# hsp-iit/roft

Hardware: AMD Instinct MI355X
Metric: tracker frames/sec per object (640x480) + ADD-S vs CPU ref (higher is better)
Workload: dtype f64; 1 GPU; BASELINE config #4: 640x480, CV_32FC2 flow grid 1, 64 objects in total, 64 per GPU (sharded by object, no data-path collective; result rows all-gathered over RCCL at N > 1), masks+poses at 5 fps with 6-frame delay, flow-aided masks, re-sync and outlier rejection on, frames submitted in batches of at most 8; objects_per_gpu=64, objects_total=64, width=640, height=480, batch_frames=8, ranks=1, backend=nccl

## Files before the change

### roft_amd/csrc/engine.hip

```cpp
#include "engine_internal.h"

namespace {
thread_local std::string g_last_error;
}

namespace roft {
namespace host {
int fail(int code, const std::string& msg)
{
    g_last_error = msg;
    return code;
}
}
}
const std::string& last_error() { return g_last_error; }

namespace roft {
int device_cu_count()
{
    static std::mutex mu;
    static std::vector<int> cus;
    int dev = 0;
    if (hipGetDevice(&dev) != hipSuccess || dev < 0) return 256;
    std::lock_guard<std::mutex> lk(mu);
// ... 635 lines not shown
            if (e->objs[obj_ids[i]]->s.track_frames > 0)
                HIP_TRY(hipMemcpyAsync(&last[i], e->arr.state.p + obj_ids[i], sizeof(ObjState), hipMemcpyDeviceToHost, s));
        HIP_TRY(hipStreamSynchronize(s));
    }
    long long meshes = 0;
    for (int i = 0; i < n; ++i) {
        const int id = obj_ids[i];
        HostObject* o = e->objs[id].get();
        if (running && o->s.track_frames > 0) {
            const ObjState& st = last[i];
            roft_object_output& out = o->last_out;
            std::memcpy(out.pose, st.belief[B_LIN0 + o->stepped_slot].mean, sizeof(double) * 13);
            std::memcpy(out.twist, st.v_mean, sizeof(double) * 6);
            out.n_flow_points = st.n_flow_points;
            out.outlier_selected = st.lane[o->stepped_lane].outlier_selected;
            out.outlier_L[0] = st.lane[o->stepped_lane].outlier_L[0];
            out.outlier_L[1] = st.lane[o->stepped_lane].outlier_L[1];
            o->last_out_valid = true;
        }
        bool mesh_uploaded = false;
        TRY(apply_object_desc(e, id, o, &descs[i], keep_mesh, &fresh[i], s, &mesh_uploaded));
        meshes += mesh_uploaded ? 1 : 0;
        o->owned.clear();
        o->s = Sched();
        o->s.frame_idx = e->frame_counter;
        o->stepped_slot = o->stepped_lane = 0;
        o->stepped_flow = nullptr;
        o->stepped_depth = nullptr;
        if (!running) continue;
        HIP_TRY(hipMemsetAsync(e->arr.planes.p + plane_offset(a, id, 0, 0), 0, sizeof(uint32_t) * (size_t)kPlaneSlotsTotal * 2 * a.plane_words, s));
        HIP_TRY(hipMemset2DAsync(e->arr.mrec.p + id, sizeof(MaskRec) * (size_t)a.n_obj, 0, sizeof(MaskRec), (size_t)2 * (kMaxBatch + 1), s));
        HIP_TRY(hipMemsetAsync(e->arr.mask_general.p + id, 0, sizeof(unsigned), s));
        HIP_TRY(hipMemset2DAsync(e->arr.npts.p + id, sizeof(int) * (size_t)a.n_obj, 0, sizeof(int), (size_t)e->T_max, s));
    }
    HIP_TRY(hipStreamSynchronize(s));
    update_mesh_maxima(e, n_obj);
    e->restart_stats.calls++;
    e->restart_stats.objects += n;
    e->restart_stats.meshes_replaced += meshes;
    return ROFT_OK;
}

int roft_engine_get_restart_stats(roft_engine* e, roft_engine_restart_stats* out)
{
    if (!e || !out) return fail(ROFT_ERR_INVALID, "null argument");
    *out = e->restart_stats;
    return ROFT_OK;
}
```

### roft_amd/csrc/engine_internal.h

```cpp
#pragma once

#include <hip/hip_runtime.h>

#include <algorithm>
#include <cfloat>
#include <chrono>
#include <cmath>
#include <cstdio>
#include <cstdlib>
#include <cstring>
#include <map>
#include <memory>
#include <mutex>
#include <string>
#include <vector>

#include "device_owned.h"
#include "roft_device.h"
#include "mesh_class.h"
#include "mesh_clusters.h"
#include "scene.h"
#include "batch_plan.h"
#include "pose_mask_gate.h"
#include "opticalflow.h"
// ... 93 lines not shown
    d.H = c.height;
    d.wpr = c.width / 32;
    d.divider = (c.width == 640) ? 2 : 4;
    d.fx = c.fx; d.fy = c.fy; d.cx = c.cx; d.cy = c.cy;
    return d;
}

inline int check_geometry(int W, int H)
{
    if (W <= 0 || H <= 0 || (W % 32) != 0 || (((size_t)W * H) % 64) != 0)
        return fail(ROFT_ERR_INVALID, "image width must be a multiple of 32 and width*height a multiple of 64");
    if ((size_t)W * H >= (1u << 24))
        return fail(ROFT_ERR_INVALID, "width*height must be < 2^24 (float-accumulated sampling index, hpp:237)");
    return ROFT_OK;
}

struct Arrays {
    EngineArrays a{};
    DevBuf<ObjParams> params;
    DevBuf<ObjState> state;
    DevBuf<FrameCtrl> ctrl;
    DevBuf<uint32_t> planes;
    DevBuf<int32_t> map;
    DevBuf<FlowRec> cand, recs;
    DevBuf<double> norms;
    DevBuf<int> npts;
    DevBuf<MaskRec> mrec;
    DevBuf<unsigned> mask_general;
    DevBuf<uint32_t> feat_pix;
    DevBuf<float> feat_depth;
    DevBuf<uint32_t> zbuf;
    DevBuf<uint32_t> zmerge;
    DevBuf<int> zcount;
    int ensure_zmerge(int n, size_t tpix)
    {
        const size_t slabs = std::max<size_t>((size_t)n, std::min<size_t>((size_t)n * kMaxOutlierParts, (size_t)std::max(device_cu_count() / 2, 1)));
        const size_t need = (size_t)kNumLin * slabs * 2 * tpix;
        if (need > zmerge.n || !zmerge.p || tpix != a.zmerge_stride || slabs != a.zmerge_slabs) {
            HIP_TRY(zmerge.ensure(need));
            a.zmerge_stride = tpix;
            a.zmerge_slabs = slabs;
        }
        HIP_TRY(zcount.ensure((size_t)kNumLin * n * 2 * kMaxOutlierParts, true));
        a.zmerge = zmerge.p;
        a.zcount = zcount.p;
        return ROFT_OK;
    }
    DevBuf<roft_object_output> log;
    DevBuf<unsigned long long> skf_started, residency;

    int alloc(int n_obj, int T, const DevCamera& cam, const DevFlowFmt& ffmt, int radius)
    {
        a.n_obj = n_obj;
        a.T = 1;
        a.cam = cam;
        a.ffmt = ffmt;
        a.plane_words = (size_t)cam.wpr * cam.H;
        const size_t npix = (size_t)cam.W * cam.H;
        a.cand_cap = ((int)((npix + radius - 1) / std::max(radius, 1)) + 9) & ~1;
        a.feat_cap = (int)(npix / 2 + 8);
        a.tile_w = cam.W / cam.divider;
        a.tile_h = cam.H / cam.divider;
        HIP_TRY(params.ensure(n_obj, true));
        HIP_TRY(state.ensure(n_obj, true));
        HIP_TRY(ctrl.ensure((size_t)n_obj * T, true));
        HIP_TRY(planes.ensure((size_t)n_obj * kPlaneSlotsTotal * 2 * a.plane_words, true));
        HIP_TRY(mrec.ensure((size_t)2 * n_obj * (kMaxBatch + 1), true));
        HIP_TRY(mask_general.ensure(n_obj, true));
        HIP_TRY(map.ensure((size_t)n_obj * npix, true));
        HIP_TRY(cand.ensure((size_t)n_obj * T * a.cand_cap));
        HIP_TRY(recs.ensure((size_t)n_obj * T * a.cand_cap));
        HIP_TRY(npts.ensure((size_t)n_obj * T, true));
        HIP_TRY(norms.ensure((size_t)n_obj * 3 * a.cand_cap));
        HIP_TRY(feat_pix.ensure((size_t)n_obj * kFeatRing * a.feat_cap));
        HIP_TRY(feat_depth.ensure((size_t)n_obj * kFeatRing * a.feat_cap));
        HIP_TRY(zbuf.ensure((size_t)2 * a.tile_w * a.tile_h));
        if (int rc = ensure_zmerge(n_obj, (size_t)a.tile_w * a.tile_h)) return rc;
        a.params = params.p; a.state = state.p; a.ctrl = ctrl.p; a.planes = planes.p; a.map = map.p;
// ... 338 lines not shown
```

### roft_amd/csrc/engine_ops.hip

```cpp
#include "op_context.h"

OpContext& roft::host::op_context()
{
    static OpContext c;
    return c;
}

namespace {

bool pose_errors_fma()
{
    static const bool fma = [] { const char* v = getenv("ROFT_POSE_ERRORS_FMA"); return !(v && v[0] == '0'); }();
    return fma;
}

}

int roft::host::pose_errors_run(PoseErrorScratch& sc, int kind, const double* d_pts, int P, const double* est_host, PoseView est_dev,
                                const double* ref_host, int n, double* out_host, hipStream_t s)
{
    const int P_pad = pose_error_padded_points(P), waves = pose_error_waves(P);
    constexpr size_t kCloudBytes = (size_t)256 << 20;
    const int per_launch = kind == ROFT_POSE_ERROR_ADDS
                               ? (int)std::min<size_t>(32768, std::max<size_t>(1, kCloudBytes / ((size_t)P_pad * 3 * sizeof(double))))
// ... 495 lines not shown
    fc.feat_read = 0;
    if (depth && mask) {
        uint8_t* d_mask;
        float* d_depth;
        TRY(c.upload(0, mask, npix, &d_mask));
        TRY(c.upload(1, depth, npix, &d_depth));
        fc.has_new_mask = 1;
        fc.new_mask = d_mask;
        fc.slot_cur = kSlotNew;
        fc.depth_cur = d_depth;
        fc.feat_write = 0;
    }
    ObjState& st = c.st;
    init_state(st);
    st.lane[0].pending_frame = 0;
    st.lane[0].pc_frame = 0;
    st.lane[0].pc_step = 1;
    for (int k = 0; k < 2; ++k) {
        PoseBelief& b = st.belief[b_alt(0, k)];
        for (int i = 0; i < 3; ++i) b.mean[6 + i] = x2[3 * k + i];
        for (int i = 0; i < 4; ++i) b.mean[9 + i] = q2[4 * k + i];
    }
    TRY(c.begin_object(a, &prm, fc));
    OutlierLaunchOpts o = o_in;
    if (tiles_out) {
        TRY(c.room(2, 2 * tpix, &o.tile_dump));
        HIP_TRY(hipMemsetAsync(o.tile_dump, 0, sizeof(float) * 2 * tpix, c.stream));
    }
    if (depth && mask) {
        launch_mask_ingest(a, 0, c.stream);
        launch_features(a, c.stream);
    }
    TRY(launch_outlier(a, 0, c.stream, nullptr, &o));
    roft_ut_params ut{1.0, 2.0, 0.0};
    launch_ukf_chain(a, ut, false, 0, c.stream);
    if (tiles_out) HIP_TRY(hipMemcpyAsync(tiles_out, o.tile_dump, sizeof(float) * 2 * tpix, hipMemcpyDeviceToHost, c.stream));
    TRY(c.read_state(a));
    for (int k = 0; k < 2; ++k) {
        if (L_out) L_out[k] = st.lane[0].outlier_L[k];
        if (samples_out) samples_out[k] = (long)st.lane[0].outlier_cnt[k];
    }
    if (selected_out) *selected_out = st.lane[0].outlier_selected;
    return ROFT_OK;
}

int roft_mesh_classify(const roft_mesh* mesh, uint8_t* flip_out, int* closed_out)
{
    if (!mesh || !mesh->verts || !mesh->tris || !has_mesh(*mesh) || !closed_out) return fail(ROFT_ERR_INVALID, "bad argument");
    std::vector<uint8_t> flip;
    *closed_out = classify_mesh(mesh->verts, mesh->n_verts, mesh->tris, mesh->n_tris, flip) ? 1 : 0;
    if (flip_out) std::memcpy(flip_out, flip.data(), (size_t)mesh->n_tris);
    return ROFT_OK;
}

int roft_render_depth(const roft_mesh* mesh, const double x[3], const double q[4], const roft_camera* cam, int divider,
                      float* tile)
{
    return roft_render_depth_mode(mesh, x, q, cam, divider, ROFT_RENDER_CONTRACT, tile);
}

int roft_render_depth_mode(const roft_mesh* mesh, const double x[3], const double q[4], const roft_camera* cam, int divider, int mode,
                           float* tile)
{
    if (!mesh || !x || !q || !cam || !tile || divider <= 0) return fail(ROFT_ERR_INVALID, "bad argument");
    if (mode != ROFT_RENDER_CONTRACT && mode != ROFT_RENDER_GL) return fail(ROFT_ERR_INVALID, "bad render mode");
    const size_t tpix = (size_t)(cam->width / divider) * (cam->height / divider);
    std::vector<float> tiles(2 * tpix);
    const double x2[6] = {x[0], x[1], x[2], x[0], x[1], x[2]};
// ... 113 lines not shown
```

### roft_amd/csrc/k_render.hip

```cpp
#include <algorithm>
#include <atomic>
#include <string>

#include "mesh_clusters.h"
#include "plane_rank.h"
#include "raster.h"

namespace roft {

namespace host { int fail(int code, const std::string& msg); }

constexpr int kFeatThreads = 1024;

#ifdef ROFT_FEAT_PROFILE
#define FTICK(i) do { __syncthreads(); if (threadIdx.x == 0) { long long _t = wall_clock64(); a.state[obj].dbg[i] = _t - f_t0; f_t0 = _t; } } while (0)
#else
#define FTICK(i) do {} while (0)
#endif

template <bool LDS>
__global__ __launch_bounds__(kFeatThreads) void features_kernel(EngineArrays a, unsigned frames_packed)
{
    ROFT_RESIDENT(a, RK_FEATURES);
    extern __shared__ __attribute__((aligned(16))) unsigned char smem[];
// ... 236 lines not shown
        const int sel = (L[0] > 2.0 * L[1]) ? 1 : 0;
        pl.outlier_selected = sel;
        pl.outlier_L[0] = L[0];
        pl.outlier_L[1] = L[1];
        for (int k = 0; k < 2; ++k) {
            double n2 = 0.0;
            for (int w = 0; w < kOutlierThreads / 64; ++w) n2 += s_cnt[k][w];
            pl.outlier_cnt[k] = n2;
        }
        s_sel = sel;
    }
    __syncthreads();
    const PoseBelief& src = st.belief[b_alt(lin, s_sel ? 1 : 0)];
    PoseBelief& dst = st.belief[c.cur_slot];
    for (int i = threadIdx.x; i < 144; i += blockDim.x) dst.cov[i] = src.cov[i];
    if (threadIdx.x < 13) dst.mean[threadIdx.x] = src.mean[threadIdx.x];
    if (roft_object_output* row = log_row(a, c, obj)) {
        if (threadIdx.x < 13) row->pose[threadIdx.x] = src.mean[threadIdx.x];
        if (threadIdx.x == 0) {
            row->outlier_selected = s_sel;
            row->outlier_L[0] = pl.outlier_L[0];
            row->outlier_L[1] = pl.outlier_L[1];
        }
    }
}

constexpr int kFusedThreads = 1024;
#ifdef ROFT_FUSED_PROFILE
#define UTICK(i) do { __syncthreads(); if (threadIdx.x == 0 && bx < 4) { long long _t = wall_clock64(); st.dbg[bx * 8 + (i)] += _t - u_t0; u_t0 = _t; } } while (0)
#else
#define UTICK(i) do {} while (0)
#endif

template <bool GL>
__global__ __launch_bounds__(kFusedThreads) void outlier_fused_kernel(EngineArrays a, int lin, int vcache_cap, int win_cap, int parts,
                                                                     int split_tris, float* tile_dump)
{
    ROFT_RESIDENT(a, RK_OUTLIER);
    extern __shared__ __attribute__((aligned(16))) unsigned char smem[];
    __shared__ long long s_hi[kFusedThreads / 64], s_lo[kFusedThreads / 64];
    __shared__ int s_cnt[kFusedThreads / 64];
    __shared__ int s_box[4];
    __shared__ int s_behind;
    __shared__ int s_last;
    __shared__ int s_settled;
    const int per = 2 * parts, lin_id = (int)blockIdx.x;
    const int obj = (lin_id / (8 * per)) * 8 + (lin_id & 7), bx = (lin_id >> 3) % per;
    if (obj >= a.n_obj) return;
    const int alt = bx / parts, part = bx % parts, tid = threadIdx.x;
    ObjState& st = a.state[obj];
    PoseLane& pl = st.lane[lin];
    if (pl.pending_frame < 0) return;
    const FrameCtrl& c = frame_ctrl(a, pl.pending_frame, obj);
    const ObjParams& prm = a.params[obj];
    const PoseBelief& bl = st.belief[b_alt(lin, alt)];
    const RenderPose P = make_pose(bl.mean + 6, bl.mean + 9);
    const int d = a.cam.divider, tw = a.tile_w, th = a.tile_h;
    const float fx = (float)(a.cam.fx / d), fy = (float)(a.cam.fy / d), cx = (float)(a.cam.cx / d), cy = (float)(a.cam.cy / d);
    const int nv = prm.n_verts, nt = prm.n_tris;
    const bool cached = GL && nv <= vcache_cap;
    float* s_v = reinterpret_cast<float*>(smem);
    uint32_t* s_z = reinterpret_cast<uint32_t*>(smem + (GL ? vertex_cache_bytes(vcache_cap) : 0));
    uint64_t* s_k = reinterpret_cast<uint64_t*>(s_z);
    if (tid < 4) s_box[tid] = (tid < 2) ? INT32_MAX : -1;
    if (tid == 0) s_behind = 0;
#ifdef ROFT_FUSED_PROFILE
    long long u_t0 = wall_clock64();
    if (tid < 8 && bx < 4) st.dbg[bx * 8 + tid] = 0;
#endif
    __syncthreads();
    auto project = [&](const float* v, float& sx, float& sy, float& z) {
        if constexpr (GL) project_vertex_gl(v, P, fx, fy, cx, cy, sx, sy, z);
        else project_vertex(v, P, fx, fy, cx, cy, sx, sy, z);
    };
    if constexpr (GL) {
        project_mesh<kFusedThreads, 4>(prm.verts, nv, cached, s_v, tw, th, s_box, &s_behind, project);
        __syncthreads();
    } else {
        if (tid < 64 && prm.n_clusters > 0) {
            const int k = tid & 7;
            const float vc[3] = {prm.box_corners[3 * k], prm.box_corners[3 * k + 1], prm.box_corners[3 * k + 2]};
            int box[4];
            const bool settled = corner_box_settles(vc, P, fx, fy, cx, cy, tw, th, box);
            if (tid == 0) {
                s_settled = settled ? 1 : 0;
                if (settled) { s_box[0] = box[0]; s_box[1] = box[1]; s_box[2] = box[2]; s_box[3] = box[3]; }
            }
        } else if (tid == 0) {
            s_settled = 1;
        }
        __syncthreads();
        if (!s_settled) {
            project_mesh<kFusedThreads, 4>(prm.verts, nv, false, s_v, tw, th, s_box, &s_behind, project);
            __syncthreads();
        }
    }
    UTICK(0);
    const int i0 = min(s_box[0], tw - 1), i1 = s_box[2];
    int j0 = min(s_box[1], th - 1), j1 = s_box[3];
    int R = parts;
    if (!GL && split_tris && parts > 1 && i1 >= i0 && j1 >= j0 && i0 >= 0 && j0 >= 0) {
        const long long w_all = i1 - i0 + 1, rows_all = j1 - j0 + 1;
// ... 95 lines not shown
                        float v_n[3] = {v[0], v[1], v[2]};
                        uint32_t w_n = w;
                        if (todo) fetch(cluster_of(base + (int)__builtin_ctzll(todo)), v_n, w_n);
                        float sx, sy, z;
                        project_vertex(v, P, fx, fy, cx, cy, sx, sy, z);
                        const int a0 = (int)(w & 63u), a1 = (int)((w >> 6) & 63u), a2 = (int)((w >> 12) & 63u);
                        const float x0 = __shfl(sx, a0, 64), y0 = __shfl(sy, a0, 64), z0 = __shfl(z, a0, 64);
                        const float x1 = __shfl(sx, a1, 64), y1 = __shfl(sy, a1, 64), z1 = __shfl(z, a1, 64);
                        const float x2 = __shfl(sx, a2, 64), y2 = __shfl(sy, a2, 64), z2 = __shfl(z, a2, 64);
                        raster_projected(x0, y0, z0, x1, y1, z1, x2, y2, z2, tw, th, js, je, rule_on ? 1 + (int)((w >> 18) & 1u) : 0, store);
                        v[0] = v_n[0]; v[1] = v_n[1]; v[2] = v_n[2];
                        w = w_n;
                    }
                }
            }
            __syncthreads();
            UTICK(2);
            if constexpr (!GL) if (split) {
                const size_t slab0 = (((size_t)lin * a.zmerge_slabs + (size_t)obj * parts + (size_t)band * G) * 2 + alt) * a.zmerge_stride;
                uint32_t* mine = a.zmerge + slab0 + (size_t)grp * 2 * a.zmerge_stride;
                int* arrivals = a.zcount + (((size_t)lin * a.n_obj + obj) * 2 + alt) * kMaxOutlierParts + band;
                for (int i = tid; i < npx; i += kFusedThreads)
                    __hip_atomic_store(&mine[i], s_z[i], __ATOMIC_RELAXED, __HIP_MEMORY_SCOPE_AGENT);
                __atomic_signal_fence(__ATOMIC_SEQ_CST);
                __builtin_amdgcn_s_waitcnt(0);
                __atomic_signal_fence(__ATOMIC_SEQ_CST);
                __syncthreads();
                if (tid == 0) {
                    const int before = __hip_atomic_fetch_add(arrivals, 1, __ATOMIC_RELAXED, __HIP_MEMORY_SCOPE_AGENT);
                    s_last = (before == G - 1) ? 1 : 0;
                    if (before == G - 1) __hip_atomic_store(arrivals, 0, __ATOMIC_RELAXED, __HIP_MEMORY_SCOPE_AGENT);
                }
                __syncthreads();
                if (!s_last) return;
                static_assert(kMaxOutlierParts <= 8, "eight slabs per pixel");
                const uint32_t* others = a.zmerge + slab0;
                const size_t slab_step = 2 * a.zmerge_stride;
                const uint32_t* op[7];
                {
                    int k = 0;
#pragma unroll
                    for (int p = 0; p < 8; ++p)
                        if (p < G && p != grp && k < 7) op[k++] = others + (size_t)p * slab_step;
                    for (; k < 7; ++k) op[k] = others;
                }
                for (int i = tid; i < npx; i += kFusedThreads) {
                    uint32_t m = s_z[i];
                    uint32_t v0, v1, v2, v3, v4, v5, v6;
                    switch (G - 1) {
                    case 1:
                        asm volatile("global_load_dword %0, %1, off sc1\n\ts_waitcnt vmcnt(0)" : "=&v"(v0) : "v"(op[0] + i) : "memory");
                        m = min(m, v0);
                        break;
                    case 2:
                        asm volatile("global_load_dword %0, %2, off sc1\n\tglobal_load_dword %1, %3, off sc1\n\ts_waitcnt vmcnt(0)"
                                     : "=&v"(v0), "=&v"(v1) : "v"(op[0] + i), "v"(op[1] + i) : "memory");
                        m = min(m, min(v0, v1));
                        break;
                    case 3:
                        asm volatile("global_load_dword %0, %3, off sc1\n\tglobal_load_dword %1, %4, off sc1\n\tglobal_load_dword %2, %5, off sc1\n\t"
                                     "s_waitcnt vmcnt(0)"
                                     : "=&v"(v0), "=&v"(v1), "=&v"(v2) : "v"(op[0] + i), "v"(op[1] + i), "v"(op[2] + i) : "memory");
                        m = min(min(m, v0), min(v1, v2));
                        break;
                    case 4:
                        asm volatile("global_load_dword %0, %4, off sc1\n\tglobal_load_dword %1, %5, off sc1\n\tglobal_load_dword %2, %6, off sc1\n\t"
                                     "global_load_dword %3, %7, off sc1\n\ts_waitcnt vmcnt(0)"
// ... 39 lines not shown
                    dep[k] = (i < n) ? fdep[i] : 0.0f;
                    pix[k] = (i < n) ? fpix[i] : 0u;
                }
#pragma unroll
                for (int k = 0; k < kBatch; ++k) {
                    if (!((dep[k] > 0) && ((double)dep[k] < 2.0))) continue;
                    const int v = (int)(pix[k] >> 16), u = (int)(pix[k] & 0xFFFFu);
                    const int tj = v / d, ti = u / d;
                    if (tj < js || tj > je || ti < i0 || ti > i1) continue;
                    if constexpr (GL) {
                        const uint64_t key = s_k[(tj - js) * win_w + (ti - i0)];
                        if ((uint32_t)(key >> 32) != kGlDepthClear) { err.add(fabsf(dep[k] - gl_resolve(key, ti, tj))); cnt += 1; }
                    } else {
                        const uint32_t b = s_z[(tj - js) * win_w + (ti - i0)];
                        if (b != kDepthEmpty) { err.add(fabsf(dep[k] - __uint_as_float(b))); cnt += 1; }
                    }
                }
            }
            __syncthreads();
            UTICK(3);
#ifdef ROFT_FUSED_PROFILE
            if (tid == 0 && bx < 4) st.dbg[bx * 8 + 4] += 1;
            if (tid == 0 && bx < 4) st.dbg[bx * 8 + 5] = (long long)win_w * 100 ;
            if (tid == 0 && bx < 4) st.dbg[bx * 8 + 6] = (long long)(j1 - j0 + 1) * 100;
#endif
        }
    }
    for (int off = 32; off > 0; off >>= 1) {
        err.hi += __shfl_down(err.hi, off, 64);
        err.lo += __shfl_down(err.lo, off, 64);
        cnt += __shfl_down(cnt, off, 64);
    }
    if ((tid & 63) == 0) { s_hi[tid >> 6] = err.hi; s_lo[tid >> 6] = err.lo; s_cnt[tid >> 6] = cnt; }
    __syncthreads();
    if (tid == 0) {
        long long hi = 0, lo = 0;
        int n2 = 0;
        for (int w = 0; w < kFusedThreads / 64; ++w) { hi += s_hi[w]; lo += s_lo[w]; n2 += s_cnt[w]; }
        pl.part_hi[alt][band] = hi;
        pl.part_lo[alt][band] = lo;
        pl.part_cnt[alt][band] = (double)n2;
        if (band == 0) pl.n_parts[alt] = R;
    }
}

static std::atomic<int> g_outlier_split{-1};
void set_outlier_split(int mode) { g_outlier_split.store(mode < 0 ? -1 : (mode ? 1 : 0), std::memory_order_relaxed); }

int launch_outlier(const EngineArrays& a, int lin, hipStream_t s, hipEvent_t stop, const OutlierLaunchOpts* opts)
{
    if (!(opts && opts->render_mode == ROFT_RENDER_GL) && a.meshes_without_clusters > 0)
        return host::fail(ROFT_ERR_STATE, "outlier test: a mesh went up without clusters (MeshLayout::kWalkClusters)");
    const size_t lds_total = kRasterLdsBudget;
    const size_t vbytes = vertex_cache_bytes(a.max_verts);
    const bool gl = opts && opts->render_mode == ROFT_RENDER_GL;
    const size_t zb = gl ? 8 : 4;
    const size_t min_win = zb * std::max(8192, a.tile_w);
    const bool cache = gl && vbytes + min_win <= lds_total && !(opts && opts->no_vertex_cache);
    const int vcache_cap = cache ? a.max_verts : 0;
    int win_cap = (int)((lds_total - (cache ? vbytes : 0)) / zb);
    (void)set_max_dynamic_lds(gl ? reinterpret_cast<const void*>(outlier_fused_kernel<true>) : reinterpret_cast<const void*>(outlier_fused_kernel<false>),
                              (int)lds_total);
    int parts = std::max(1, std::min(kMaxOutlierParts, device_cu_count() / (2 * std::max(a.n_obj, 1))));
    if (a.outlier_parts > 0) parts = std::min(a.outlier_parts, kMaxOutlierParts);
    if (opts && opts->parts > 0) parts = std::min(opts->parts, kMaxOutlierParts);
    if (opts && opts->parts < 0) parts = std::max(1, parts / -opts->parts);
    static const int split_env = getenv("ROFT_OUTLIER_SPLIT") ? atoi(getenv("ROFT_OUTLIER_SPLIT")) : -1;
    const int forced = g_outlier_split.load(std::memory_order_relaxed) >= 0 ? g_outlier_split.load(std::memory_order_relaxed) : split_env;
    int split = (opts && opts->split >= 0) ? opts->split : (forced >= 0 ? forced : 1);
    if (parts <= 1 || !a.zmerge || (size_t)a.n_obj * parts > a.zmerge_slabs) split = 0;
    if (gl) split = 0;
    const int lds_parts = split ? 1 : parts;
    const size_t win_need = zb * std::max((size_t)a.tile_w, ((size_t)a.tile_w * a.tile_h + lds_parts - 1) / lds_parts + (size_t)a.tile_w);
    const size_t lds = std::min(lds_total, (((cache ? vbytes : 0) + win_need + 15) & ~(size_t)15));
    win_cap = std::min(win_cap, (int)((lds - (cache ? vbytes : 0)) / zb));
// ... 17 lines not shown
```

### roft_amd/csrc/k_ukf.hip

```cpp
#include "roft_device.h"

#pragma clang fp contract(fast)

namespace roft {

#ifdef ROFT_UKF_PROFILE
#define TICK(L, i) do { __syncthreads(); if (threadIdx.x == 0) { long long _t = clock64(); (L).dbg[i] += _t - (L).t0; (L).t0 = _t; } } while (0)
#else
#define TICK(L, i) do {} while (0)
#endif

constexpr int kUkfThreads = 256;

__device__ __forceinline__ void wave_sync()
{
    __builtin_amdgcn_fence(__ATOMIC_RELEASE, "wavefront");
    __builtin_amdgcn_wave_barrier();
    __builtin_amdgcn_fence(__ATOMIC_ACQUIRE, "wavefront");
}

__device__ __forceinline__ void quat_mul(const double a[4], const double b[4], double o[4])
{
    const double w = a[0] * b[0] - a[1] * b[1] - a[2] * b[2] - a[3] * b[3];
    const double x = a[0] * b[1] + a[1] * b[0] + a[2] * b[3] - a[3] * b[2];
// ... 865 lines not shown
    else chol_solve_rows<12>(L.aug, L.rc, L.Pxy, L.K);
    __syncthreads();
    TICK(L, 25);
    if (lane < 12 * m) {
        const int i = lane / m, j = lane % m;
        double s = 0.0;
        for (int k = 0; k < m; ++k) s += L.K[i * m + k] * L.Py[k * m + j];
        L.KPy[i * m + j] = s;
    } else if (lane >= 192 && lane < 192 + 12) {
        const int i = lane - 192;
        double s = 0.0;
        for (int k = 0; k < m; ++k) s += L.K[i * m + k] * L.innov[k];
        L.Kin[i] = s;
    }
    __syncthreads();
    TICK(L, 26);
    if (lane < 144) {
        const int i = lane / 12, j = lane % 12;
        double s = 0.0;
        for (int k = 0; k < m; ++k) s += L.KPy[i * m + k] * L.K[j * m + k];
        out->cov[lane] = L.cov[lane] - s;
    } else if (lane >= 192 && lane < 192 + 9) {
        out->mean[lane - 192] = L.mean[lane - 192] + L.Kin[lane - 192];
    } else if (lane == 192 + 9) {
        double qo[4];
        quat_boxplus(L.mean + 9, L.Kin + 9, qo);
        for (int i = 0; i < 4; ++i) out->mean[9 + i] = qo[i];
    }
    __syncthreads();
    TICK(L, 12);
    return 0;
}

__device__ bool ukf_one_step(const EngineArrays& a, const FrameCtrl& c, int obj, int step, const UtTable& ut, UkfLds& L)
{
    ObjState& st = a.state[obj];
    struct {
        int op, src, do_predict, n_corr, type0, type1, dst0, dst1, twist_slot;
    } sd;
    {
        const StepDesc& d = c.steps[step];
        sd.op = d.op; sd.src = d.src; sd.do_predict = d.do_predict; sd.n_corr = d.n_corr;
        sd.type0 = d.type[0]; sd.type1 = d.type[1]; sd.dst0 = d.dst[0]; sd.dst1 = d.dst[1]; sd.twist_slot = d.twist_slot;
    }
    if (!sd.op) return true;
    const ObjParams& prm = a.params[obj];
    const int lane = threadIdx.x;
    const int lin = c.lane, cur = c.cur_slot;

#ifdef ROFT_UKF_PROFILE
    if (lane < 32) L.dbg[lane] = 0;
    if (lane == 0) L.t0 = clock64();
    __syncthreads();
#endif
    const PoseBelief& src = st.belief[sd.src];
    for (int i = lane; i < 144; i += kUkfThreads) L.cov[i] = src.cov[i];
    if (lane < 13) L.mean[lane] = src.mean[lane];
    static_assert(offsetof(ObjParams, R_q) == 21 * sizeof(double), "L.par mirrors the head of ObjParams");
    if (lane >= 160 && lane < 184) L.par[lane - 160] = reinterpret_cast<const double*>(&prm)[lane - 160];
    if (lane >= 192) {
        const int i = lane - 192;
        if (a.handoff) {
            const int want = c.frame_idx - ((c.frame_idx - sd.twist_slot) & (kTwistRing - 1)) + 1;
            if (lane == 192) {
                const long long t0 = wall_clock64();
                unsigned spins = 0;
                int timed_out = 0;
                while (__hip_atomic_load(&st.twist_tag[sd.twist_slot], __ATOMIC_RELAXED, __HIP_MEMORY_SCOPE_AGENT) < want) {
                    __builtin_amdgcn_s_sleep(1);
                    if ((++spins & 4095u) == 0u && wall_clock64() - t0 > 200000000ll) {
                        if (a.dev_error) __hip_atomic_store(a.dev_error, ROFT_DEV_ERROR_TWIST_WAIT, __ATOMIC_RELAXED, __HIP_MEMORY_SCOPE_SYSTEM);
                        timed_out = 1;
                        break;
                    }
                }
                L.twist_timeout = timed_out;
            }
            __atomic_signal_fence(__ATOMIC_SEQ_CST);
            if (i < 6) L.meas[i] = __longlong_as_double((long long)__hip_atomic_load(
                reinterpret_cast<const unsigned long long*>(&st.twist_hist[sd.twist_slot][i]), __ATOMIC_RELAXED, __HIP_MEMORY_SCOPE_AGENT));
        } else if (i < 6) {
            L.meas[i] = st.twist_hist[sd.twist_slot][i];
        }
        if (i >= 6 && i < 13) L.meas[i] = (i < 9) ? c.pose_x[i - 6] : c.pose_q[i - 9];
    }
    __syncthreads();
    if (a.handoff && L.twist_timeout) return false;

    TICK(L, 0);
    if (sd.do_predict) {
        ukf_predict(L, prm, c.dt, ut, st.warm_V[cur][0], &st.warm_age[cur][0], a.ukf_chol_guard);
        PoseBelief& pr = st.belief[B_PRED + lin];
// ... 28 lines not shown
    if (lane < 32) st.dbg[lane] = L.dbg[lane];
#endif
    return true;
}

#ifndef PRIO_UKF
#define PRIO_UKF 3
#endif
#ifdef UKF_WAVES_PER_EU
__attribute__((amdgpu_waves_per_eu(UKF_WAVES_PER_EU, UKF_WAVES_PER_EU)))
#endif
__global__ __launch_bounds__(kUkfThreads) void ukf_chain_kernel(EngineArrays a, UtTable ut, int first_segment, int lin)
{
    ROFT_RESIDENT(a, RK_UKF_CHAIN);
    __shared__ UkfLds L;
    uint4 tab_word = make_uint4(0u, 0u, 0u, 0u);
    if ((int)threadIdx.x < kUkfTabWords) tab_word = reinterpret_cast<const uint4*>(&g_ukf_tab)[threadIdx.x];
    __builtin_amdgcn_s_setprio(PRIO_UKF);
#ifdef ROFT_UKF_WALL
    const long long w_entry = wall_clock64();
    __shared__ unsigned s_ticket;
    if (threadIdx.x == 0) {
        s_ticket = atomicAdd(reinterpret_cast<unsigned*>(&a.state[0].dbg[30 + 0]) + lin, 1u);
        long long* rec = a.state[(s_ticket / a.n_obj) % a.n_obj].dbg + lin * 8;
        const long long now = wall_clock64();
        atomicMax(reinterpret_cast<unsigned long long*>(&rec[0]), (unsigned long long)((1ll << 62) - now));
        atomicMax(reinterpret_cast<unsigned long long*>(&rec[1]), (unsigned long long)now);
    }
    __syncthreads();
#endif
    const int obj = blockIdx.x;
    ObjState& st = a.state[obj];
    PoseLane& pl = st.lane[lin];
    int t = first_segment ? 0 : pl.pc_frame, step = first_segment ? 0 : pl.pc_step;
    if (t >= a.T) return;
    const int vote_lane = threadIdx.x & 63;
    const unsigned mine = (unsigned)__ballot(vote_lane < a.T && frame_ctrl(a, vote_lane, obj).lane == lin);
    if ((mine >> t) == 0u) {
        if (threadIdx.x == 0) { pl.pending_frame = -1; pl.pc_frame = a.T; pl.pc_step = 0; }
        return;
    }
    if (!first_segment && pl.pending_frame >= 0) {
        const FrameCtrl& pc = frame_ctrl(a, pl.pending_frame, obj);
        double Lk[2];
        for (int k = 0; k < 2; ++k) {
            long long hi = 0, lo = 0;
            double n2 = 0.0;
            for (int p = 0; p < pl.n_parts[k]; ++p) { hi += pl.part_hi[k][p]; lo += pl.part_lo[k][p]; n2 += pl.part_cnt[k][p]; }
            const double e = LikelihoodSum::value(hi, lo);
            Lk[k] = (n2 == 0.0) ? 1.7976931348623157e308 : (e / n2) / 1.0;
            if (threadIdx.x == 0) { pl.outlier_L[k] = Lk[k]; pl.outlier_cnt[k] = n2; }
        }
        const double L0 = Lk[0], L1 = Lk[1];
        const int sel = (L0 > 2.0 * L1) ? 1 : 0;
        const PoseBelief& src = st.belief[b_alt(lin, sel)];
        PoseBelief& dst = st.belief[pc.cur_slot];
        for (int i = threadIdx.x; i < 144; i += kUkfThreads) dst.cov[i] = src.cov[i];
        if (threadIdx.x < 13) dst.mean[threadIdx.x] = src.mean[threadIdx.x];
        roft_object_output* row = log_row(a, pc, obj);
        if (row && threadIdx.x < 13) row->pose[threadIdx.x] = src.mean[threadIdx.x];
        if (threadIdx.x == 0) {
            pl.outlier_selected = sel;
            if (row) { row->outlier_selected = sel; row->outlier_L[0] = L0; row->outlier_L[1] = L1; }
        }
        __syncthreads();
    }
    static_assert(kUkfTabWords <= kUkfThreads, "one 16-byte word of the tables per thread");
    if ((int)threadIdx.x < kUkfTabWords) reinterpret_cast<uint4*>(&L.tab)[threadIdx.x] = tab_word;
    for (int i = threadIdx.x; i < 100; i += kUkfThreads) L.Q[i] = 0.0;
    __syncthreads();
    bool pending = false;
    __shared__ FrameCtrl s_c;
    int staged = -1;
#ifdef ROFT_UKF_WALL
    const long long w_t0 = wall_clock64();
    int w_steps = 0;
    long long* w_rec = a.state[(s_ticket / a.n_obj) % a.n_obj].dbg + lin * 8;
#endif
    while (t < a.T) {
        if (!((mine >> t) & 1u)) { ++t; step = 0; continue; }
        if (staged != t) {
            __syncthreads();
            stage_ctrl(&s_c, frame_ctrl(a, t, obj));
            staged = t;
            __syncthreads();
        }
        const FrameCtrl& c = s_c;
        if (step == 0 && threadIdx.x == 0) {
            pl.outlier_selected = -1;
            if (roft_object_output* row0 = log_row(a, c, obj)) row0->outlier_selected = -1;
        }
        if (step >= c.n_steps) { ++t; step = 0; continue; }
#ifdef ROFT_UKF_WALL
        const long long w_s0 = wall_clock64();
#endif
        if (c.steps[step].op && !ukf_one_step(a, c, obj, step, ut, L)) {
            __syncthreads();
            t = a.T;
            step = 0;
            pending = false;
            break;
        }
#ifdef ROFT_UKF_WALL
        if (threadIdx.x == 0 && w_steps == 0) {
            atomicAdd(reinterpret_cast<unsigned long long*>(&st.dbg[26]), (unsigned long long)(w_s0 - w_entry));
            atomicAdd(reinterpret_cast<unsigned long long*>(&st.dbg[27]), (unsigned long long)(wall_clock64() - w_s0));
            atomicAdd(reinterpret_cast<unsigned long long*>(&st.dbg[19]), 1ull);
        }
        if (threadIdx.x == 0 && w_steps > 0) {
            const long long d = wall_clock64() - w_s0;
            const int bin = d < 1800 ? 0 : (d < 2200 ? 1 : (d < 3000 ? 2 : 3));
            atomicAdd(reinterpret_cast<unsigned long long*>(&st.dbg[20 + bin]), 1ull);
            if (bin == 3) atomicAdd(reinterpret_cast<unsigned long long*>(&st.dbg[24]), (unsigned long long)d);
            if (bin == 3) atomicAdd(reinterpret_cast<unsigned long long*>(&st.dbg[25]), (unsigned long long)(c.steps[step].n_corr * 100 + c.steps[step].type[0]));
        }
        ++w_steps;
#endif
        __syncthreads();
        pending = (step == c.outlier_step);
        ++step;
        if (pending) break;
    }
#ifdef ROFT_UKF_WALL
    if (threadIdx.x == 0) {
        const long long w_t1 = wall_clock64();
        atomicAdd(reinterpret_cast<unsigned long long*>(&st.dbg[28]), (unsigned long long)(w_t1 - w_t0));
        atomicAdd(reinterpret_cast<unsigned long long*>(&st.dbg[29]), (unsigned long long)w_steps);
        atomicMax(reinterpret_cast<unsigned long long*>(&w_rec[2]), (unsigned long long)w_t1);
        atomicMax(reinterpret_cast<unsigned long long*>(&w_rec[3]), (unsigned long long)w_steps);
        atomicAdd(reinterpret_cast<unsigned long long*>(&w_rec[4]), (unsigned long long)w_steps);
        atomicAdd(reinterpret_cast<unsigned long long*>(&w_rec[5]), 1ull);
        if (w_steps > 0) atomicMax(reinterpret_cast<unsigned long long*>(&w_rec[6]), (unsigned long long)((w_t1 - w_t0) / w_steps));
        if (w_steps > 0) atomicMax(reinterpret_cast<unsigned long long*>(&w_rec[7]), (unsigned long long)(w_t1 - w_t0));
    }
#endif
    if (threadIdx.x == 0) {
        pl.pending_frame = pending ? t : -1;
        pl.pc_frame = t;
        pl.pc_step = step;
    }
}

void launch_ukf_chain(const EngineArrays& a, roft_ut_params ut, bool first_segment, int lin, hipStream_t s, hipEvent_t stop)
{
    UtTable tab;
    for (int k = 0; k < 3; ++k) tab.w[k] = ut_weights(18 + 3 * k, ut);
    hipExtLaunchKernelGGL(ukf_chain_kernel, dim3(a.n_obj), dim3(kUkfThreads), 0, s, nullptr, stop, 0, a, tab,
                          first_segment ? 1 : 0, lin);
}

// ... 2 lines not shown
```

### roft_amd/csrc/roft_device.h

```cpp
#pragma once

#include <hip/hip_runtime.h>
#include <hip/hip_ext.h>
#include <stdint.h>

#include "../../include/roft_engine.h"

namespace roft {

constexpr int kWave = 64;
constexpr int kNumLin = 2;
constexpr int kNumBelief = 9;
constexpr int kMaxBatch = ROFT_MAX_BATCH_FRAMES;
constexpr int kTwistRing = 64;
constexpr int kMaxFlowHist = ROFT_MAX_FLOW_CHASE;
constexpr int kMaxOutlierParts = 8;
constexpr int kMaxSteps = 10;
constexpr int kPlaneSlots = 64;
constexpr int kFeatRing = 12;

enum BeliefSlot { B_LIN0 = 0, B_LIN1 = 1, B_PRED = 2 , B_ALT0 = 4 , B_ALT1 = 5 ,
                  B_SPARE = 8, B_CORR = B_LIN0  };
__host__ __device__ inline int b_alt(int lane, int k) { return B_ALT0 + 2 * lane + k; }

// ... 127 lines not shown
    {
        const double xs = fmin((double)x, 256.0) * 4294967296.0;
        const double fl = floor(xs);
        hi += (long long)fl;
        lo += (long long)((xs - fl) * 4294967296.0);
    }
    __host__ __device__ static double value(long long hi, long long lo) { return (double)hi * (1.0 / 4294967296.0) + (double)lo * (1.0 / 4294967296.0 / 4294967296.0); }
};

struct EngineArrays {
    int n_obj;
    DevCamera cam;
    DevFlowFmt ffmt;
    ObjParams* params;
    ObjState* state;
    int T;
    FrameCtrl* ctrl;
    uint32_t* planes;
    MaskRec* mrec;
    const MaskRec* mrec_carry;
    int slot_new;
    int slot_prev0;
    unsigned* mask_general;
    int32_t* map;
    FlowRec* cand;
    FlowRec* recs;
    int* npts;
    double* norms;
    uint32_t* feat_pix;
    float* feat_depth;
    uint32_t* zbuf;
    uint32_t* zmerge;
    int* zcount;
    size_t zmerge_stride;
    size_t zmerge_slabs;
    int cand_cap, feat_cap;
    size_t plane_words;
    int tile_w, tile_h;
    int max_tris, max_verts;
    int meshes_without_clusters;
    double ukf_chol_guard;
    double ukf_chol_guard_bil;
    roft_object_output* out_log;
    int log_cap;
    int mask_wgs;
    int outlier_parts;
    int* dev_error;
    int handoff;
    unsigned long long* skf_started;
    unsigned long long* residency;
    unsigned long long* k1_span;
};

enum ResidencyKernel { RK_MASK_FRAME = 0, RK_MASK_INGEST, RK_MASK_GENERAL, RK_FLOW_MEASURE, RK_SKF_CHAIN, RK_FEATURES, RK_UKF_CHAIN, RK_OUTLIER,
                       RK_MASK_FRAME_EMPTY ,
                       RK_MASK_FRESH, RK_MASK_FRESH_EMPTY , RK_COUNT };
#ifdef ROFT_RESIDENCY
struct ResidencyTimer {
    unsigned long long* p;
    long long t0;
    __device__ ResidencyTimer(unsigned long long* base, int kid) : p(base ? base + 2 * kid : nullptr), t0(wall_clock64()) {}
    __device__ ~ResidencyTimer()
    {
        if (p && threadIdx.x == 0) { atomicAdd(p, (unsigned long long)(wall_clock64() - t0)); atomicAdd(p + 1, 1ull); }
    }
    __device__ void rekind(unsigned long long* base, int kid) { if (base) p = base + 2 * kid; }
// ... 190 lines not shown
```

Baseline: 1.772 million object-frames/s.

## Resolve outlier selection in last-arriving outlier block; prefetch UKF entry state

The outlier kernel now counts finished blocks per object and lane with a new arrival counter. The last block to arrive reduces the partial likelihoods, picks the alternative, and writes the chosen belief and log row, so the UKF chain no longer does this reduction and copy on entry. The UKF kernel also preloads all of the batch's frame-control blocks and the two linearisation beliefs into shared memory once, instead of staging each frame's control block and reading beliefs from global memory per step. This adds cross-block atomics and cache-bypassing (sc1) loads whose correctness depends on memory ordering. The counter must also be reset on restart, which the change handles.

Measured after the change: 1.781 million object-frames/s (median of 3 runs). Within noise of the previous version (+0.5%).

```diff
diff --git a/roft_amd/csrc/engine.hip b/roft_amd/csrc/engine.hip
--- a/roft_amd/csrc/engine.hip
+++ b/roft_amd/csrc/engine.hip
@@ -691,6 +691,7 @@
         HIP_TRY(hipMemset2DAsync(e->arr.mrec.p + id, sizeof(MaskRec) * (size_t)a.n_obj, 0, sizeof(MaskRec), (size_t)2 * (kMaxBatch + 1), s));
         HIP_TRY(hipMemsetAsync(e->arr.mask_general.p + id, 0, sizeof(unsigned), s));
         HIP_TRY(hipMemset2DAsync(e->arr.npts.p + id, sizeof(int) * (size_t)a.n_obj, 0, sizeof(int), (size_t)e->T_max, s));
+        HIP_TRY(hipMemset2DAsync(e->arr.ocount.p + id, sizeof(int) * (size_t)a.n_obj, 0, sizeof(int), (size_t)kNumLin, s));
     }
     HIP_TRY(hipStreamSynchronize(s));
     update_mesh_maxima(e, n_obj);
diff --git a/roft_amd/csrc/engine_internal.h b/roft_amd/csrc/engine_internal.h
--- a/roft_amd/csrc/engine_internal.h
+++ b/roft_amd/csrc/engine_internal.h
@@ -149,6 +149,7 @@
     DevBuf<uint32_t> zbuf;
     DevBuf<uint32_t> zmerge;
     DevBuf<int> zcount;
+    DevBuf<int> ocount;
     int ensure_zmerge(int n, size_t tpix)
     {
         const size_t slabs = std::max<size_t>((size_t)n, std::min<size_t>((size_t)n * kMaxOutlierParts, (size_t)std::max(device_cu_count() / 2, 1)));
@@ -159,8 +160,10 @@
             a.zmerge_slabs = slabs;
         }
         HIP_TRY(zcount.ensure((size_t)kNumLin * n * 2 * kMaxOutlierParts, true));
+        HIP_TRY(ocount.ensure((size_t)kNumLin * n, true));
         a.zmerge = zmerge.p;
         a.zcount = zcount.p;
+        a.ocount = ocount.p;
         return ROFT_OK;
     }
     DevBuf<roft_object_output> log;
diff --git a/roft_amd/csrc/engine_ops.hip b/roft_amd/csrc/engine_ops.hip
--- a/roft_amd/csrc/engine_ops.hip
+++ b/roft_amd/csrc/engine_ops.hip
@@ -551,8 +551,6 @@
         launch_features(a, c.stream);
     }
     TRY(launch_outlier(a, 0, c.stream, nullptr, &o));
-    roft_ut_params ut{1.0, 2.0, 0.0};
-    launch_ukf_chain(a, ut, false, 0, c.stream);
     if (tiles_out) HIP_TRY(hipMemcpyAsync(tiles_out, o.tile_dump, sizeof(float) * 2 * tpix, hipMemcpyDeviceToHost, c.stream));
     TRY(c.read_state(a));
     for (int k = 0; k < 2; ++k) {
diff --git a/roft_amd/csrc/k_render.hip b/roft_amd/csrc/k_render.hip
--- a/roft_amd/csrc/k_render.hip
+++ b/roft_amd/csrc/k_render.hip
@@ -292,6 +292,20 @@
 #define UTICK(i) do {} while (0)
 #endif
 
+__device__ __forceinline__ bool test_arrive(int* arrivals, int total, int* s_flag)
+{
+    if (threadIdx.x == 0) {
+        const int before = __hip_atomic_fetch_add(arrivals, 1, __ATOMIC_RELAXED, __HIP_MEMORY_SCOPE_AGENT);
+        *s_flag = (before == total - 1) ? 1 : 0;
+        if (before == total - 1) __hip_atomic_store(arrivals, 0, __ATOMIC_RELAXED, __HIP_MEMORY_SCOPE_AGENT);
+    }
+    __syncthreads();
+    return *s_flag != 0;
+}
+
+constexpr int kBeliefDoubles = (int)(sizeof(PoseBelief) / sizeof(double));
+static_assert(sizeof(PoseBelief) == 157 * sizeof(double) && offsetof(PoseBelief, mean) == 0, "a belief is copied as 157 doubles, the mean first");
+
 template <bool GL>
 __global__ __launch_bounds__(kFusedThreads) void outlier_fused_kernel(EngineArrays a, int lin, int vcache_cap, int win_cap, int parts,
                                                                      int split_tris, float* tile_dump)
@@ -304,6 +318,7 @@
     __shared__ int s_behind;
     __shared__ int s_last;
     __shared__ int s_settled;
+    __shared__ int s_decide;
     const int per = 2 * parts, lin_id = (int)blockIdx.x;
     const int obj = (lin_id / (8 * per)) * 8 + (lin_id & 7), bx = (lin_id >> 3) % per;
     if (obj >= a.n_obj) return;
@@ -312,6 +327,8 @@
     PoseLane& pl = st.lane[lin];
     if (pl.pending_frame < 0) return;
     const FrameCtrl& c = frame_ctrl(a, pl.pending_frame, obj);
+    int cur_slot = c.cur_slot, frame_idx = c.frame_idx;
+    int* const obj_arrivals = a.ocount + (size_t)lin * a.n_obj + obj;
     const ObjParams& prm = a.params[obj];
     const PoseBelief& bl = st.belief[b_alt(lin, alt)];
     const RenderPose P = make_pose(bl.mean + 6, bl.mean + 9);
@@ -328,6 +345,9 @@
     long long u_t0 = wall_clock64();
     if (tid < 8 && bx < 4) st.dbg[bx * 8 + tid] = 0;
 #endif
+    asm volatile("" : "+v"(cur_slot), "+v"(frame_idx));
+    cur_slot = __builtin_amdgcn_readfirstlane(cur_slot);
+    frame_idx = __builtin_amdgcn_readfirstlane(frame_idx);
     __syncthreads();
     auto project = [&](const float* v, float& sx, float& sy, float& z) {
         if constexpr (GL) project_vertex_gl(v, P, fx, fy, cx, cy, sx, sy, z);
@@ -489,7 +509,10 @@
                     if (before == G - 1) __hip_atomic_store(arrivals, 0, __ATOMIC_RELAXED, __HIP_MEMORY_SCOPE_AGENT);
                 }
                 __syncthreads();
-                if (!s_last) return;
+                if (!s_last) {
+                    (void)test_arrive(obj_arrivals, per, &s_decide);
+                    return;
+                }
                 static_assert(kMaxOutlierParts <= 8, "eight slabs per pixel");
                 const uint32_t* others = a.zmerge + slab0;
                 const size_t slab_step = 2 * a.zmerge_stride;
@@ -595,15 +618,62 @@
         cnt += __shfl_down(cnt, off, 64);
     }
     if ((tid & 63) == 0) { s_hi[tid >> 6] = err.hi; s_lo[tid >> 6] = err.lo; s_cnt[tid >> 6] = cnt; }
+    double bel0 = 0.0, bel1 = 0.0;
+    if (tid < kBeliefDoubles) {
+        bel0 = reinterpret_cast<const double*>(&st.belief[b_alt(lin, 0)])[tid];
+        bel1 = reinterpret_cast<const double*>(&st.belief[b_alt(lin, 1)])[tid];
+    }
     __syncthreads();
     if (tid == 0) {
         long long hi = 0, lo = 0;
         int n2 = 0;
         for (int w = 0; w < kFusedThreads / 64; ++w) { hi += s_hi[w]; lo += s_lo[w]; n2 += s_cnt[w]; }
-        pl.part_hi[alt][band] = hi;
-        pl.part_lo[alt][band] = lo;
-        pl.part_cnt[alt][band] = (double)n2;
-        if (band == 0) pl.n_parts[alt] = R;
+        __hip_atomic_store(&pl.part_hi[alt][band], hi, __ATOMIC_RELAXED, __HIP_MEMORY_SCOPE_AGENT);
+        __hip_atomic_store(&pl.part_lo[alt][band], lo, __ATOMIC_RELAXED, __HIP_MEMORY_SCOPE_AGENT);
+        __hip_atomic_store(reinterpret_cast<long long*>(&pl.part_cnt[alt][band]), __double_as_longlong((double)n2), __ATOMIC_RELAXED, __HIP_MEMORY_SCOPE_AGENT);
+        if (band == 0) __hip_atomic_store(&pl.n_parts[alt], R, __ATOMIC_RELAXED, __HIP_MEMORY_SCOPE_AGENT);
+        __atomic_signal_fence(__ATOMIC_SEQ_CST);
+        __builtin_amdgcn_s_waitcnt(0);
+        __atomic_signal_fence(__ATOMIC_SEQ_CST);
+    }
+    if (!test_arrive(obj_arrivals, per, &s_decide)) return;
+    __syncthreads();
+    roft_object_output* const row = a.out_log ? a.out_log + (size_t)(frame_idx % a.log_cap) * a.n_obj + obj : nullptr;
+    if (tid < 64) {
+        const int k = (tid >> 3) & 1, p = tid & 7;
+        static_assert(kMaxOutlierParts == 8, "eight lanes per alternative");
+        unsigned long long w_hi, w_lo, w_cnt;
+        int np;
+        asm volatile("global_load_dwordx2 %0, %4, off sc1\n\tglobal_load_dwordx2 %1, %5, off sc1\n\tglobal_load_dwordx2 %2, %6, off sc1\n\t"
+                     "global_load_dword %3, %7, off sc1\n\ts_waitcnt vmcnt(0)"
+                     : "=&v"(w_hi), "=&v"(w_lo), "=&v"(w_cnt), "=&v"(np)
+                     : "v"(&pl.part_hi[k][p]), "v"(&pl.part_lo[k][p]), "v"(&pl.part_cnt[k][p]), "v"(&pl.n_parts[k]) : "memory");
+        long long hi = (p < np) ? (long long)w_hi : 0ll, lo = (p < np) ? (long long)w_lo : 0ll;
+        double n2 = (p < np) ? __longlong_as_double((long long)w_cnt) : 0.0;
+        for (int off = 4; off > 0; off >>= 1) {
+            hi += __shfl_xor(hi, off, 64);
+            lo += __shfl_xor(lo, off, 64);
+            n2 += __shfl_xor(n2, off, 64);
+        }
+        const double e = LikelihoodSum::value(hi, lo);
+        const double Lk = (n2 == 0.0) ? 1.7976931348623157e308 : (e / n2) / 1.0;
+        const double L0 = __shfl(Lk, 0, 64), L1 = __shfl(Lk, 8, 64);
+        const double n0 = __shfl(n2, 0, 64), n1 = __shfl(n2, 8, 64);
+        if (tid == 0) {
+            const int sel = (L0 > 2.0 * L1) ? 1 : 0;
+            s_decide = sel;
+            pl.outlier_L[0] = L0; pl.outlier_L[1] = L1;
+            pl.outlier_cnt[0] = n0; pl.outlier_cnt[1] = n1;
+            pl.outlier_selected = sel;
+            pl.pending_frame = -1;
+            if (row) { row->outlier_selected = sel; row->outlier_L[0] = L0; row->outlier_L[1] = L1; }
+        }
+    }
+    __syncthreads();
+    if (tid < kBeliefDoubles) {
+        const double v = s_decide ? bel1 : bel0;
+        reinterpret_cast<double*>(&st.belief[cur_slot])[tid] = v;
+        if (row && tid < 13) row->pose[tid] = v;
     }
 }
 
diff --git a/roft_amd/csrc/k_ukf.hip b/roft_amd/csrc/k_ukf.hip
--- a/roft_amd/csrc/k_ukf.hip
+++ b/roft_amd/csrc/k_ukf.hip
@@ -921,7 +921,9 @@
     return 0;
 }
 
-__device__ bool ukf_one_step(const EngineArrays& a, const FrameCtrl& c, int obj, int step, const UtTable& ut, UkfLds& L)
+constexpr int kEntryBeliefStride = 160;
+__device__ bool ukf_one_step(const EngineArrays& a, const FrameCtrl& c, int obj, int step, const UtTable& ut, UkfLds& L,
+                             const double* entry_beliefs = nullptr)
 {
     ObjState& st = a.state[obj];
     struct {
@@ -942,11 +944,19 @@
     if (lane == 0) L.t0 = clock64();
     __syncthreads();
 #endif
-    const PoseBelief& src = st.belief[sd.src];
-    for (int i = lane; i < 144; i += kUkfThreads) L.cov[i] = src.cov[i];
-    if (lane < 13) L.mean[lane] = src.mean[lane];
     static_assert(offsetof(ObjParams, R_q) == 21 * sizeof(double), "L.par mirrors the head of ObjParams");
-    if (lane >= 160 && lane < 184) L.par[lane - 160] = reinterpret_cast<const double*>(&prm)[lane - 160];
+    static_assert(B_LIN0 == 0 && B_LIN1 == 1 && offsetof(PoseBelief, mean) == 0 && offsetof(PoseBelief, cov) == 13 * sizeof(double),
+                  "the entry's copies: slot s at entry_beliefs + s * kEntryBeliefStride, the mean first");
+    if (entry_beliefs && (sd.src == B_LIN0 || sd.src == B_LIN1)) {
+        const double* pre = entry_beliefs + sd.src * kEntryBeliefStride;
+        for (int i = lane; i < 144; i += kUkfThreads) L.cov[i] = pre[13 + i];
+        if (lane < 13) L.mean[lane] = pre[lane];
+    } else {
+        const PoseBelief& src = st.belief[sd.src];
+        for (int i = lane; i < 144; i += kUkfThreads) L.cov[i] = src.cov[i];
+        if (lane < 13) L.mean[lane] = src.mean[lane];
+        if (lane >= 160 && lane < 184) L.par[lane - 160] = reinterpret_cast<const double*>(&prm)[lane - 160];
+    }
     if (lane >= 192) {
         const int i = lane - 192;
         if (a.handoff) {
@@ -1041,46 +1051,54 @@
     const int obj = blockIdx.x;
     ObjState& st = a.state[obj];
     PoseLane& pl = st.lane[lin];
-    int t = first_segment ? 0 : pl.pc_frame, step = first_segment ? 0 : pl.pc_step;
+    constexpr int kCtrlWords = (int)(sizeof(FrameCtrl) / 16);
+    static_assert(kMaxBatch * kCtrlWords <= 2 * kUkfThreads, "two words of the batch's control blocks per thread");
+    __shared__ FrameCtrl s_ctrl[kMaxBatch];
+    int t = 0, step = 0;
+    if (!first_segment) { t = pl.pc_frame; step = pl.pc_step; }
+    const int vote_lane = threadIdx.x & 63;
+    int vote_field = -1;
+    if (vote_lane < a.T) vote_field = frame_ctrl(a, vote_lane, obj).lane;
+    const int n_ctrl_words = min(a.T, kMaxBatch) * kCtrlWords;
+    const int cw0 = threadIdx.x, cw1 = threadIdx.x + kUkfThreads;
+    uint4 ctrl_word0 = make_uint4(0u, 0u, 0u, 0u), ctrl_word1 = make_uint4(0u, 0u, 0u, 0u);
+    if (cw0 < n_ctrl_words) ctrl_word0 = reinterpret_cast<const uint4*>(&frame_ctrl(a, cw0 / kCtrlWords, obj))[cw0 % kCtrlWords];
+    if (cw1 < n_ctrl_words) ctrl_word1 = reinterpret_cast<const uint4*>(&frame_ctrl(a, cw1 / kCtrlWords, obj))[cw1 % kCtrlWords];
+    constexpr int kBeliefDoubles = (int)(sizeof(PoseBelief) / sizeof(double));
+    static_assert(kBeliefDoubles <= kEntryBeliefStride && 2 * kEntryBeliefStride <= 13 * kCols, "both slots fit L.Y");
+    double entry_b0 = 0.0, entry_b1 = 0.0, entry_par = 0.0;
+    if ((int)threadIdx.x < kBeliefDoubles) {
+        entry_b0 = reinterpret_cast<const double*>(&st.belief[B_LIN0])[threadIdx.x];
+        entry_b1 = reinterpret_cast<const double*>(&st.belief[B_LIN1])[threadIdx.x];
+    } else if (threadIdx.x >= 160 && threadIdx.x < 184) {
+        entry_par = reinterpret_cast<const double*>(&a.params[obj])[threadIdx.x - 160];
+    }
+    asm volatile("" : "+v"(t), "+v"(step), "+v"(vote_field), "+v"(tab_word.x), "+v"(tab_word.y), "+v"(tab_word.z), "+v"(tab_word.w),
+                      "+v"(ctrl_word0.x), "+v"(ctrl_word0.y), "+v"(ctrl_word0.z), "+v"(ctrl_word0.w),
+                      "+v"(ctrl_word1.x), "+v"(ctrl_word1.y), "+v"(ctrl_word1.z), "+v"(ctrl_word1.w),
+                      "+v"(entry_b0), "+v"(entry_b1), "+v"(entry_par));
+    t = __builtin_amdgcn_readfirstlane(t);
+    step = __builtin_amdgcn_readfirstlane(step);
     if (t >= a.T) return;
-    const int vote_lane = threadIdx.x & 63;
-    const unsigned mine = (unsigned)__ballot(vote_lane < a.T && frame_ctrl(a, vote_lane, obj).lane == lin);
+    const unsigned mine = (unsigned)__ballot(vote_field == lin);
     if ((mine >> t) == 0u) {
         if (threadIdx.x == 0) { pl.pending_frame = -1; pl.pc_frame = a.T; pl.pc_step = 0; }
         return;
     }
-    if (!first_segment && pl.pending_frame >= 0) {
-        const FrameCtrl& pc = frame_ctrl(a, pl.pending_frame, obj);
-        double Lk[2];
-        for (int k = 0; k < 2; ++k) {
-            long long hi = 0, lo = 0;
-            double n2 = 0.0;
-            for (int p = 0; p < pl.n_parts[k]; ++p) { hi += pl.part_hi[k][p]; lo += pl.part_lo[k][p]; n2 += pl.part_cnt[k][p]; }
-            const double e = LikelihoodSum::value(hi, lo);
-            Lk[k] = (n2 == 0.0) ? 1.7976931348623157e308 : (e / n2) / 1.0;
-            if (threadIdx.x == 0) { pl.outlier_L[k] = Lk[k]; pl.outlier_cnt[k] = n2; }
-        }
-        const double L0 = Lk[0], L1 = Lk[1];
-        const int sel = (L0 > 2.0 * L1) ? 1 : 0;
-        const PoseBelief& src = st.belief[b_alt(lin, sel)];
-        PoseBelief& dst = st.belief[pc.cur_slot];
-        for (int i = threadIdx.x; i < 144; i += kUkfThreads) dst.cov[i] = src.cov[i];
-        if (threadIdx.x < 13) dst.mean[threadIdx.x] = src.mean[threadIdx.x];
-        roft_object_output* row = log_row(a, pc, obj);
-        if (row && threadIdx.x < 13) row->pose[threadIdx.x] = src.mean[threadIdx.x];
-        if (threadIdx.x == 0) {
-            pl.outlier_selected = sel;
-            if (row) { row->outlier_selected = sel; row->outlier_L[0] = L0; row->outlier_L[1] = L1; }
-        }
-        __syncthreads();
-    }
     static_assert(kUkfTabWords <= kUkfThreads, "one 16-byte word of the tables per thread");
     if ((int)threadIdx.x < kUkfTabWords) reinterpret_cast<uint4*>(&L.tab)[threadIdx.x] = tab_word;
+    if (cw0 < n_ctrl_words) reinterpret_cast<uint4*>(s_ctrl)[cw0] = ctrl_word0;
+    if (cw1 < n_ctrl_words) reinterpret_cast<uint4*>(s_ctrl)[cw1] = ctrl_word1;
+    if ((int)threadIdx.x < kBeliefDoubles) {
+        L.Y[threadIdx.x] = entry_b0;
+        L.Y[kEntryBeliefStride + threadIdx.x] = entry_b1;
+    } else if (threadIdx.x >= 160 && threadIdx.x < 184) {
+        L.par[threadIdx.x - 160] = entry_par;
+    }
     for (int i = threadIdx.x; i < 100; i += kUkfThreads) L.Q[i] = 0.0;
     __syncthreads();
     bool pending = false;
-    __shared__ FrameCtrl s_c;
-    int staged = -1;
+    const double* entry_beliefs = L.Y;
 #ifdef ROFT_UKF_WALL
     const long long w_t0 = wall_clock64();
     int w_steps = 0;
@@ -1088,13 +1106,7 @@
 #endif
     while (t < a.T) {
         if (!((mine >> t) & 1u)) { ++t; step = 0; continue; }
-        if (staged != t) {
-            __syncthreads();
-            stage_ctrl(&s_c, frame_ctrl(a, t, obj));
-            staged = t;
-            __syncthreads();
-        }
-        const FrameCtrl& c = s_c;
+        const FrameCtrl& c = s_ctrl[t];
         if (step == 0 && threadIdx.x == 0) {
             pl.outlier_selected = -1;
             if (roft_object_output* row0 = log_row(a, c, obj)) row0->outlier_selected = -1;
@@ -1103,7 +1115,8 @@
 #ifdef ROFT_UKF_WALL
         const long long w_s0 = wall_clock64();
 #endif
-        if (c.steps[step].op && !ukf_one_step(a, c, obj, step, ut, L)) {
+        const bool walks = c.steps[step].op != 0;
+        if (walks && !ukf_one_step(a, c, obj, step, ut, L, entry_beliefs)) {
             __syncthreads();
             t = a.T;
             step = 0;
@@ -1125,6 +1138,7 @@
         }
         ++w_steps;
 #endif
+        if (walks) entry_beliefs = nullptr;
         __syncthreads();
         pending = (step == c.outlier_step);
         ++step;
diff --git a/roft_amd/csrc/roft_device.h b/roft_amd/csrc/roft_device.h
--- a/roft_amd/csrc/roft_device.h
+++ b/roft_amd/csrc/roft_device.h
@@ -183,6 +183,7 @@
     uint32_t* zbuf;
     uint32_t* zmerge;
     int* zcount;
+    int* ocount;
     size_t zmerge_stride;
     size_t zmerge_slabs;
     int cand_cap, feat_cap;
```
